# limacv/VideoLoop3D

Hardware: AMD Instinct MI355X
Metric: rendered Mpix/s (fwd+bwd) D=32 planes 720p (higher is better)
Workload: dtype f32; 1 GPU; cfg3 stage-2 MPV render fwd+bwd: D=32 planes, T=50 frames, 720x1280, mpv convention, plane stack (D,T,H,W,4) f32 resident in HBM; parallelism=single GPU, variant=0

## Files before the change

### profiles/ab_inproc.py

```python
#!/usr/bin/env python3
import argparse
import os
import statistics
import sys

sys.path.insert(0, os.path.dirname(os.path.dirname(os.path.abspath(__file__))))
import torch

ap = argparse.ArgumentParser()
ap.add_argument("--variants", default="0,3")
ap.add_argument("--rounds", type=int, default=6)
ap.add_argument("--reps", type=int, default=4)
ap.add_argument("--stack-scale", type=float, default=1.0)
ap.add_argument("--reg", action="store_true", help="smoothness regularisers on (the REG backward)")
ap.add_argument("--dtype", default="f32")
ap.add_argument("--D", type=int, default=32)
ap.add_argument("--T", type=int, default=50)
ap.add_argument("--H", type=int, default=720)
ap.add_argument("--W", type=int, default=1280)
a = ap.parse_args()

import __graft_entry__ as ge
ge.build()
from videoloop3d_amd import synth
from videoloop3d_amd.render import RenderSpec, render_planes, render_planes_with_smoothness
from videoloop3d_amd.utils_mpi import compute_homography, make_depths

dev = torch.device("cuda:0")
D, T, H, W = a.D, a.T, a.H, a.W
Hs, Ws = int(H * a.stack_scale), int(W * a.stack_scale)
ref_e, Kr, tar_e, Kt = synth.make_cameras(H, W)
homos = compute_homography(ref_e[None], Kr[None], tar_e[None], Kt[None], torch.tensor([0., 0., 1.]).expand(1, D, 3),
                           make_depths(D, 1.0, 100.0).flip(0)[None])[0]
shift = torch.tensor([[1.0, 0, (Ws - W) // 2], [0, 1.0, (Hs - H) // 2], [0, 0, 1.0]])
homos_d = (shift @ homos).to(dev)
stack = synth.make_plane_stack(D, T, Hs, Ws, seed=2, device=dev, dtype=torch.float16 if a.dtype == "f16" else torch.float32).requires_grad_(True)
g = synth.hash_uniform((T, H, W, 3), seed=5, device=dev) - 0.5
variants = [int(v, 0) for v in a.variants.split(",")]
ev = lambda: torch.cuda.Event(enable_timing=True)
res = [([], []) for _ in variants]


def once(v):
    spec = RenderSpec.mpv(variant=v)
    e0, e1, e2 = ev(), ev(), ev()
    e0.record()
    if a.reg:
        rgb, alpha, sums = render_planes_with_smoothness(stack, homos_d, H, W, spec)
        obj = (rgb * g).sum() + 1e-6 * sums.sum()
        e1.record()
        (gs,) = torch.autograd.grad(obj, stack)
    else:
        rgb, alpha = render_planes(stack, homos_d, H, W, spec)
        e1.record()
        (gs,) = torch.autograd.grad(rgb, stack, g)
    e2.record()
    torch.cuda.synchronize()
    once.last = gs
    return e0.elapsed_time(e1), e1.elapsed_time(e2)


g_first = None
for v in variants:
    once(v)
    if g_first is None:
        g_first = once.last.clone() if T <= 4 else None
    elif T <= 4:
        print(f"variant {v:#x}: gradient bits equal to variant {variants[0]:#x}: {torch.equal(g_first, once.last)}")
for r in range(a.rounds):
    for i, v in enumerate(variants):
        for _ in range(a.reps):
            f, b = once(v)
            res[i][0].append(f)
            res[i][1].append(b)
print(f"D={D} T={T} {H}x{W} stack {Hs}x{Ws} {a.dtype} reg={a.reg}: {a.rounds} rounds x {a.reps} reps, interleaved")
bmed = [statistics.median(b) for _, b in res]
for i, v in enumerate(variants):
    f, b = res[i]
    print(f"variant {v:#6x}  fwd median {statistics.median(f):7.3f} min {min(f):7.3f}   bwd median {bmed[i]:7.3f} min {min(b):7.3f} ms"
          + (f"   bwd vs leg 0: {100.0 * (bmed[i] / bmed[0] - 1.0):+6.2f} %" if i else ""))
spread = max([abs(bmed[i] - bmed[j]) for i in range(len(variants)) for j in range(i) if variants[i] == variants[j]], default=None)
if spread is not None:
    print(f"spread (backward medians of the legs that repeat a variant): {spread:.3f} ms = {100.0 * spread / bmed[0]:.2f} %; a gain counts from 3x that: {3 * spread:.3f} ms")
```

### videoloop3d_amd/csrc/vl3d_render_core.h

```cpp
#pragma once
#include <stddef.h>
#include "vl3d_common.h"
#include "vl3d_bake_rule.h"

#include "vl3d_adam.h"
#include "vl3d_render_bwd_choice.h"

#ifndef VL3D_HS
#define VL3D_HS 9
#define VL3D_HN 9
#endif

namespace vl3d_render_detail {

#ifndef VL3D_PAIR_MIN_WAVES
#define VL3D_PAIR_MIN_WAVES 4
#endif
#ifndef VL3D_FWD2X_MIN_WAVES
#define VL3D_FWD2X_MIN_WAVES 4
#endif

#ifdef VL3D_REG_ABLATE
#define VL3D_REGAB(bit) ((VL3D_REG_ABLATE & (bit)) != 0)
#else
// ... 565 lines not shown
    const float S = dot3p(Gr, a.rgb[pix * 3 + 0], Gg, a.rgb[pix * 3 + 1], Gb, a.rgb[pix * 3 + 2], gA * a.alpha[pix]);
    const float gN1 = a.g_asum ? a.g_asum[pix * 2 + 0] : 0.0f, gN2 = a.g_asum ? 2.0f * a.g_asum[pix * 2 + 1] : 0.0f;
    const unsigned fl = a.g_reg ? a.reg_flags[(size_t)y * a.W + x] : 0u;
    float Tr = 1.0f, P = 0.0f;
    const TapStep st = make_tap_step<F16>(a.Hs, a.Ws), gst = make_tap_step<false>(a.Hs, a.Ws);
    const float gL = MASK ? a.g_label[pix] : 0.0f;
    const size_t mframe = (size_t)a.Hs * a.Ws;
    for (int d = 0; d < a.D; ++d, plane += (size_t)a.T * a.Hs * a.Ws * TEXB, gplane += (size_t)a.T * a.Hs * a.Ws * TEXB) {
        const Taps2 tp = make_taps2<COORD, BORDER>(a.homos + VL3D_HS * d, px, py, a.Hs, a.Ws, a.sx, a.sy, a.ox, a.oy, plane_cull(a, d), UvNoise{a.uv_seed, d});
        if (tp.cov == 0.0f) continue;
        typename TapVal<F16, ORDER>::type tv[4];
        f4 pre;
        load_taps2<F16>(plane, tp, st, tv);
        const f4 o = shade2<ORDER, RACT, AACT>(tp, tv, &pre);
        const float q = dot3p(Gr, o.x, Gg, o.y, Gb, o.z, gA);
        const float w = o.w * Tr;
        if constexpr (MASK) {
            float mt[4];
            load_mask_taps(a.mask + ((size_t)d * a.T + t) * mframe, tp.off, gst, mt);
            const float sm = act_fwd<VL3D_ACT_SIGMOID>(mask_blend(mt, tp.w));
            const float gm = gL * w * (sm * (1.0f - sm));
            float *gmp = a.g_mask + ((size_t)d * a.T + t) * mframe + (tp.off >> 4);
#pragma unroll
            for (int i = 0; i < 4; ++i)
                if (tp.w[i] != 0.0f) atomicAdd(gmp + ((i & 1) ? (gst.dx >> 4) : 0u) + ((i & 2) ? (gst.dy >> 4) : 0u), gm * tp.w[i]);
        }
        P = fmaf(w, q, P);
        const float om = 1.0f - o.w;
        const float behind = (om > 1e-12f) ? (S - P) * fast_rcp(om) : 0.0f;
        f4 go = f4{w * Gr, w * Gg, w * Gb, fmaf(Tr, q, -behind) + fmaf(gN2, o.w, gN1)};
        Tr *= om;
        if (a.g_reg) {
            const f4 gx = f4{a.g_reg[0], a.g_reg[0], a.g_reg[0], a.g_reg[2]}, gy = f4{a.g_reg[1], a.g_reg[1], a.g_reg[1], a.g_reg[3]};
            const size_t idx = (((((size_t)(d >> 2) * a.T + t) * a.H + y) * a.W + x) << 2) + (d & 3);
            const unsigned w_left = x >= 1 ? a.reg_signs[idx - 4] : REG_ZERO, w_up = y >= 1 ? a.reg_signs[idx - 4 * (size_t)a.W] : REG_ZERO;
            go += reg_grad(a.reg_signs[idx], w_left, w_up, (fl & 12u) ? a.reg_patch[idx] : 0u, fl, gx, gy);
        }
        if constexpr (ORDER == VL3D_ACT_POST)
            go = f4{go.x * act_bwd<RACT>(pre.x, o.x), go.y * act_bwd<RACT>(pre.y, o.y), go.z * act_bwd<RACT>(pre.z, o.z),
                    go.w * act_bwd<AACT>(pre.w, o.w)};
#pragma unroll
        for (int i = 0; i < 4; ++i) {
            if (tp.w[i] != 0.0f) {
                f4 c = go * tp.w[i];
                if constexpr (ORDER == VL3D_ACT_PRE || ORDER == VL3D_ACT_BAKED) {
                    const f4 sv = tv[i];
                    c = f4{c.x * act_bwd<RACT>(sv.x, act_fwd<RACT>(sv.x)), c.y * act_bwd<RACT>(sv.y, act_fwd<RACT>(sv.y)),
                           c.z * act_bwd<RACT>(sv.z, act_fwd<RACT>(sv.z)), c.w * act_bwd<AACT>(sv.w, act_fwd<AACT>(sv.w))};
                }
                atomic_add_grad_texel<F16>(gplane, (size_t)tp.off + ((i & 1) ? gst.dx : 0u) + ((i & 2) ? gst.dy : 0u), c);
            }
        }
    }
}

__device__ __forceinline__ int xcd_remap(int b, int nb) {
    const int q = nb >> 3, r = nb & 7, xcd = b & 7, k = b >> 3;
    return (xcd < r ? xcd * (q + 1) : r * (q + 1) + (xcd - r) * q) + k;
}

template <int COORD, bool CAMS = false>
__global__ __launch_bounds__(256) void cull_fwd_plan_k(RenderArgs a, int TY, int tiles_x, int tiles_y, unsigned long long *masks) {
    const int i = blockIdx.x * 256 + threadIdx.x;
    if (i >= tiles_x * tiles_y * a.D) return;
    const int d = i % a.D, tile = i / a.D, tile_x = tile % tiles_x, tile_y = tile / tiles_x;
    const int x0 = tile_x * 64, x1 = min(x0 + 63, a.W - 1), y0 = tile_y * TY, y1 = min(y0 + TY - 1, a.H - 1);
    const float *h = a.homos + VL3D_HS * d;
    if constexpr (CAMS) {
        h += (size_t)blockIdx.y * a.D * VL3D_HS;
        masks += (size_t)blockIdx.y * tiles_x * tiles_y * 2;
    }
    float tnx = 1e30f, txx = -1e30f, tny = 1e30f, txy = -1e30f;
    for (int c = 0; c < 4; ++c) {
        const float cx = (float)a.col0 + a.pc + (float)((c & 1) ? x1 : x0), cy = (float)a.row0 + a.pc + (float)((c & 2) ? y1 : y0);
        const float X = h[0] * cx + h[1] * cy + h[2], Y = h[3] * cx + h[4] * cy + h[5], Z = h[6] * cx + h[7] * cy + h[8];
        const float ctx = texel_coord<COORD>(X / Z, (float)a.Ws / 2.0f, (float)(a.Ws - 1), a.sx, a.ox);
        const float cty = texel_coord<COORD>(Y / Z, (float)a.Hs / 2.0f, (float)(a.Hs - 1), a.sy, a.oy);
        tnx = fminf(tnx, ctx); txx = fmaxf(txx, ctx); tny = fminf(tny, cty); txy = fmaxf(txy, cty);
    }
    if (box_touches_kept_quad(a, d, tnx, txx, tny, txy)) atomicOr(masks + (size_t)tile * 2 + (d >> 6), 1ull << (d & 63));
}

template <int COORD>
void launch_cull_fwd_plan(const RenderArgs &a, int TY, int tiles_x, int tiles_y, hipStream_t s) {
    auto *masks = const_cast<unsigned long long *>(a.cull_masks);
    (void)hipMemsetAsync(masks, 0, (size_t)tiles_x * tiles_y * 16, s);
    const int n = tiles_x * tiles_y * a.D;
    hipLaunchKernelGGL((cull_fwd_plan_k<COORD>), dim3((n + 255) / 256), dim3(256), 0, s, a, TY, tiles_x, tiles_y, masks);
}
template <int COORD>
void launch_cull_fwd_plan_cams(const RenderArgs &a, int n_cams, int TY, int tiles_x, int tiles_y, hipStream_t s) {
    auto *masks = const_cast<unsigned long long *>(a.cull_masks);
    (void)hipMemsetAsync(masks, 0, (size_t)n_cams * tiles_x * tiles_y * 16, s);
    const int n = tiles_x * tiles_y * a.D;
    hipLaunchKernelGGL((cull_fwd_plan_k<COORD, true>), dim3((n + 255) / 256, n_cams), dim3(256), 0, s, a, TY, tiles_x, tiles_y, masks);
}

struct PlaneList {
    unsigned long long m0, m1;
    __device__ __forceinline__ PlaneList(const unsigned long long *cull_masks, int tile) {
        typedef const __attribute__((address_space(4))) unsigned long long *cu64_p;
        const cu64_p mk = (cu64_p)(cull_masks + (size_t)tile * 2);
        m0 = mk[0]; m1 = mk[1];
    }
    __device__ __forceinline__ int next() {
        int d = -1;
        if (m0) { d = __builtin_ctzll(m0); m0 &= m0 - 1; }
        else if (m1) { d = 64 + __builtin_ctzll(m1); m1 &= m1 - 1; }
        return d;
    }
};

template <int COORD, int BORDER, int ORDER, int RACT, int AACT, int TY, bool SWZ, bool F16, bool CULL = false, bool MASK = false>
__global__ __launch_bounds__(64 * TY) void render_fwd2_k(RenderArgs a, int tiles_x, int tiles_y) {
    static_assert(!(MASK && (CULL || F16)), "the loop-mask channel: dense fp32 stage-1 stacks");
    int b = blockIdx.x;
    if constexpr (SWZ) b = xcd_remap(b, gridDim.x);
    const int tile_x = b % tiles_x, rest = b / tiles_x;
    const int tile_y = rest % tiles_y, t = rest / tiles_y;
    const int x = tile_x * 64 + (threadIdx.x & 63);
    const int y = tile_y * TY + (threadIdx.x >> 6);
    if (x >= a.W || y >= a.H) return;
    const float px = (float)(a.col0 + x) + a.pc, py = (float)(a.row0 + y) + a.pc;
    const size_t frame_b = (size_t)a.Hs * a.Ws * (F16 ? 8 : 16);
    const size_t plane_stride_b = (size_t)a.Tstride * frame_b;
    const char *plane = reinterpret_cast<const char *>(a.stack) + (size_t)t * frame_b;
    float Tr = 1.0f, cr = 0.f, cg = 0.f, cb = 0.f, A = 0.f, n1 = 0.f, n2 = 0.f;
    const TapStep st = make_tap_step<F16>(a.Hs, a.Ws);
    typedef typename TapVal<F16, ORDER>::type tapv_t;
    tapv_t vA[4], vB[4];
    float mA[4] = {0.f, 0.f, 0.f, 0.f}, mB[4] = {0.f, 0.f, 0.f, 0.f}, lab = 0.f;
    const float *mplane = MASK ? a.mask + (size_t)t * a.Hs * a.Ws : nullptr;
    const size_t mplane_stride = (size_t)a.T * a.Hs * a.Ws;
#define VL3D_COMPOSITE(T_, V_, M_)                                    \
    {                                                                 \
        const f4 o = shade2<ORDER, RACT, AACT>(T_, V_);               \
        const float w = o.w * Tr;                                     \
        cr += w * o.x; cg += w * o.y; cb += w * o.z; A += w;          \
        n1 += o.w; n2 = fmaf(o.w, o.w, n2);                           \
        Tr *= (1.0f - o.w);                                           \
        if constexpr (MASK) lab = fmaf(w, act_fwd<VL3D_ACT_SIGMOID>(mask_blend(M_, T_.w)), lab);      \
    }
    if constexpr (CULL) {
        PlaneList list(a.cull_masks, tile_y * tiles_x + tile_x);
        auto fetch = [&](int d, Taps2 &t, tapv_t *v) {
            float h[VL3D_HN];
            load_uniform(a.homos + VL3D_HS * d, h);
            t = make_taps2<COORD, BORDER>(h, px, py, a.Hs, a.Ws, a.sx, a.sy, a.ox, a.oy, plane_cull(a, d), UvNoise{a.uv_seed, d});
            load_taps2<F16>(plane + (size_t)d * plane_stride_b, t, st, v);
            asm volatile("" ::: "memory");
        };
        int dA = list.next();
        if (dA >= 0) {
            Taps2 tA, tB;
            fetch(dA, tA, vA);
            for (;;) {
                const int dB = list.next();
                fetch(dB < 0 ? dA : dB, tB, vB);
                VL3D_COMPOSITE(tA, vA, mA)
                if (dB < 0) break;
                const int dC = list.next();
                fetch(dC < 0 ? dB : dC, tA, vA);
                VL3D_COMPOSITE(tB, vB, mB)
                if (dC < 0) break;
                dA = dC;
            }
        }
    } else {
    const QuadCull noq = QuadCull{nullptr, 0, 0, 0.f, 0.f, 0.f, 0.f, 0};
    Taps2 tA = make_taps2<COORD, BORDER>(a.homos, px, py, a.Hs, a.Ws, a.sx, a.sy, a.ox, a.oy, noq, UvNoise{a.uv_seed, 0}), tB = tA;
    load_taps2<F16>(plane, tA, st, vA);
    if constexpr (MASK) load_mask_taps(mplane, tA.off, st, mA);
    for (int d = 0;; d += 2) {
        {
            const int dn = min(d + 1, a.D - 1);
            float h[VL3D_HN];
            load_uniform(a.homos + VL3D_HS * dn, h);
            tB = make_taps2<COORD, BORDER>(h, px, py, a.Hs, a.Ws, a.sx, a.sy, a.ox, a.oy, noq, UvNoise{a.uv_seed, dn});
            load_taps2<F16>(plane + (size_t)dn * plane_stride_b, tB, st, vB);
            if constexpr (MASK) load_mask_taps(mplane + (size_t)dn * mplane_stride, tB.off, st, mB);
            asm volatile("" ::: "memory");
        }
        VL3D_COMPOSITE(tA, vA, mA)
        if (d + 1 >= a.D) break;
        {
            const int dn = min(d + 2, a.D - 1);
            float h[VL3D_HN];
            load_uniform(a.homos + VL3D_HS * dn, h);
            tA = make_taps2<COORD, BORDER>(h, px, py, a.Hs, a.Ws, a.sx, a.sy, a.ox, a.oy, noq, UvNoise{a.uv_seed, dn});
            load_taps2<F16>(plane + (size_t)dn * plane_stride_b, tA, st, vA);
            if constexpr (MASK) load_mask_taps(mplane + (size_t)dn * mplane_stride, tA.off, st, mA);
            asm volatile("" ::: "memory");
        }
        VL3D_COMPOSITE(tB, vB, mB)
        if (d + 2 >= a.D) break;
    }
    }
#undef VL3D_COMPOSITE
    const size_t pix = ((size_t)t * a.H + y) * a.W + x;
    a.rgb[pix * 3 + 0] = cr; a.rgb[pix * 3 + 1] = cg; a.rgb[pix * 3 + 2] = cb;
    a.alpha[pix] = A;
    if (a.asum) { a.asum[pix * 2 + 0] = n1; a.asum[pix * 2 + 1] = n2; }
    if constexpr (MASK) a.label[pix] = lab;
}

template <int COORD, int BORDER, int ORDER, int RACT, int AACT, int TY, bool F16, bool CULL = false>
__global__ __launch_bounds__(64 * TY, VL3D_FWD2X_MIN_WAVES) void render_fwd2x_k(RenderArgs a, int tiles_x, int tiles_y) {
    const int b = xcd_remap(blockIdx.x, gridDim.x);
    const int tile_x = b % tiles_x, rest = b / tiles_x;
    const int tile_y = rest % tiles_y, t0 = (rest / tiles_y) * 2;
    const bool has1 = t0 + 1 < a.T;
    const int x = tile_x * 64 + (threadIdx.x & 63);
    const int y = tile_y * TY + (threadIdx.x >> 6);
    if (x >= a.W || y >= a.H) return;
    const float px = (float)(a.col0 + x) + a.pc, py = (float)(a.row0 + y) + a.pc;
    const size_t frame_b = (size_t)a.Hs * a.Ws * (F16 ? 8 : 16);
    const size_t plane_stride_b = (size_t)a.Tstride * frame_b;
    const char *plane0 = reinterpret_cast<const char *>(a.stack) + (size_t)t0 * frame_b;
    const char *plane1 = plane0 + (has1 ? frame_b : 0);
    float Tr0 = 1.0f, cr0 = 0.f, cg0 = 0.f, cb0 = 0.f, A0 = 0.f, n10 = 0.f, n20 = 0.f;
    float Tr1 = 1.0f, cr1 = 0.f, cg1 = 0.f, cb1 = 0.f, A1 = 0.f, n11 = 0.f, n21 = 0.f;
    const TapStep st = make_tap_step<F16>(a.Hs, a.Ws);
    typedef typename TapVal<F16, ORDER>::type tapv_t;
    tapv_t vA0[4], vA1[4], vB0[4], vB1[4];
#define VL3D_COMPOSITE2(T_, V0_, V1_)                                        \
    {                                                                        \
        const f4 o0 = shade2<ORDER, RACT, AACT>(T_, V0_);                    \
        const f4 o1 = shade2<ORDER, RACT, AACT>(T_, V1_);                    \
        const float w0 = o0.w * Tr0, w1 = o1.w * Tr1;                        \
        cr0 += w0 * o0.x; cg0 += w0 * o0.y; cb0 += w0 * o0.z; A0 += w0;      \
        cr1 += w1 * o1.x; cg1 += w1 * o1.y; cb1 += w1 * o1.z; A1 += w1;      \
        n10 += o0.w; n20 = fmaf(o0.w, o0.w, n20);                            \
        n11 += o1.w; n21 = fmaf(o1.w, o1.w, n21);                            \
        Tr0 *= (1.0f - o0.w); Tr1 *= (1.0f - o1.w);                          \
    }
    if constexpr (CULL) {
        PlaneList list(a.cull_masks, tile_y * tiles_x + tile_x);
        auto fetch = [&](int d, Taps2 &t, tapv_t *v0, tapv_t *v1) {
            float h[VL3D_HN];
            load_uniform(a.homos + VL3D_HS * d, h);
            t = make_taps2<COORD, BORDER>(h, px, py, a.Hs, a.Ws, a.sx, a.sy, a.ox, a.oy, plane_cull(a, d));
            load_taps2<F16>(plane0 + (size_t)d * plane_stride_b, t, st, v0);
            load_taps2<F16>(plane1 + (size_t)d * plane_stride_b, t, st, v1);
            asm volatile("" ::: "memory");
        };
        int dA = list.next();
        if (dA >= 0) {
            Taps2 tA, tB;
            fetch(dA, tA, vA0, vA1);
            for (;;) {
                const int dB = list.next();
                fetch(dB < 0 ? dA : dB, tB, vB0, vB1);
                VL3D_COMPOSITE2(tA, vA0, vA1)
                if (dB < 0) break;
                const int dC = list.next();
                fetch(dC < 0 ? dB : dC, tA, vA0, vA1);
                VL3D_COMPOSITE2(tB, vB0, vB1)
                if (dC < 0) break;
                dA = dC;
            }
        }
    } else {
    Taps2 tA = make_taps2<COORD, BORDER>(a.homos, px, py, a.Hs, a.Ws, a.sx, a.sy, a.ox, a.oy), tB = tA;
    load_taps2<F16>(plane0, tA, st, vA0);
    load_taps2<F16>(plane1, tA, st, vA1);
    for (int d = 0;; d += 2) {
        {
            const int dn = min(d + 1, a.D - 1);
            float h[VL3D_HN];
            load_uniform(a.homos + VL3D_HS * dn, h);
            tB = make_taps2<COORD, BORDER>(h, px, py, a.Hs, a.Ws, a.sx, a.sy, a.ox, a.oy);
            load_taps2<F16>(plane0 + (size_t)dn * plane_stride_b, tB, st, vB0);
            load_taps2<F16>(plane1 + (size_t)dn * plane_stride_b, tB, st, vB1);
            asm volatile("" ::: "memory");
        }
        VL3D_COMPOSITE2(tA, vA0, vA1)
        if (d + 1 >= a.D) break;
        {
            const int dn = min(d + 2, a.D - 1);
            float h[VL3D_HN];
            load_uniform(a.homos + VL3D_HS * dn, h);
            tA = make_taps2<COORD, BORDER>(h, px, py, a.Hs, a.Ws, a.sx, a.sy, a.ox, a.oy);
            load_taps2<F16>(plane0 + (size_t)dn * plane_stride_b, tA, st, vA0);
            load_taps2<F16>(plane1 + (size_t)dn * plane_stride_b, tA, st, vA1);
            asm volatile("" ::: "memory");
        }
        VL3D_COMPOSITE2(tB, vB0, vB1)
        if (d + 2 >= a.D) break;
    }
    }
#undef VL3D_COMPOSITE2
    size_t pix = ((size_t)t0 * a.H + y) * a.W + x;
    a.rgb[pix * 3 + 0] = cr0; a.rgb[pix * 3 + 1] = cg0; a.rgb[pix * 3 + 2] = cb0;
    a.alpha[pix] = A0;
    if (a.asum) { a.asum[pix * 2 + 0] = n10; a.asum[pix * 2 + 1] = n20; }
    if (has1) {
        pix += (size_t)a.H * a.W;
        a.rgb[pix * 3 + 0] = cr1; a.rgb[pix * 3 + 1] = cg1; a.rgb[pix * 3 + 2] = cb1;
        a.alpha[pix] = A1;
        if (a.asum) { a.asum[pix * 2 + 0] = n11; a.asum[pix * 2 + 1] = n21; }
    }
}

template <int COORD, int BORDER, int ORDER, int RACT, int AACT, bool F16>
void launch_fwd2x(const RenderArgs &a, hipStream_t s) {
    constexpr int TY = 8;
    const int tiles_x = (a.W + 63) / 64, tiles_y = (a.H + TY - 1) / TY;
    const dim3 grid((unsigned)(tiles_x * tiles_y * ((a.T + 1) / 2))), block(64 * TY);
    if (a.quad_keep && a.cull_masks) {
        launch_cull_fwd_plan<COORD>(a, TY, tiles_x, tiles_y, s);
        hipLaunchKernelGGL((render_fwd2x_k<COORD, BORDER, ORDER, RACT, AACT, TY, F16, true>), grid, block, 0, s, a, tiles_x, tiles_y);
        return;
    }
    hipLaunchKernelGGL((render_fwd2x_k<COORD, BORDER, ORDER, RACT, AACT, TY, F16>), grid, block, 0, s, a, tiles_x, tiles_y);
}

template <int COORD, int BORDER, int ORDER, int RACT, int AACT, int TY, bool SWZ, bool F16 = false>
void launch_fwd2(const RenderArgs &a, hipStream_t s) {
    const int tiles_x = (a.W + 63) / 64, tiles_y = (a.H + TY - 1) / TY;
    if (a.quad_keep && a.cull_masks) {
        launch_cull_fwd_plan<COORD>(a, TY, tiles_x, tiles_y, s);
        hipLaunchKernelGGL((render_fwd2_k<COORD, BORDER, ORDER, RACT, AACT, TY, SWZ, F16, true>), dim3((unsigned)(tiles_x * tiles_y * a.T)),
                           dim3(64 * TY), 0, s, a, tiles_x, tiles_y);
        return;
    }
    hipLaunchKernelGGL((render_fwd2_k<COORD, BORDER, ORDER, RACT, AACT, TY, SWZ, F16>), dim3((unsigned)(tiles_x * tiles_y * a.T)),
                       dim3(64 * TY), 0, s, a, tiles_x, tiles_y);
}

constexpr int RW = 64;
constexpr int PLAN_HDR = 16;
constexpr int PLAN_REC = 12;
__host__ __device__ inline int plan_win_off(int D) { return (PLAN_HDR + PLAN_REC * D + 3) & ~3; }

template <int COORD>
__device__ void texel_homography(const float *h, int Hs, int Ws, float sx, float sy, float ox, float oy, double M[9]) {
    double ax, ay, bx, by;
    if constexpr (COORD == VL3D_COORD_UTILS_MPI) { ax = (double)(Ws - 1) / Ws; ay = (double)(Hs - 1) / Hs; bx = by = 0.0; }
    else { ax = sx; ay = sy; bx = ox; by = oy; }
    for (int j = 0; j < 3; ++j) {
        M[0 + j] = ax * h[0 + j] + bx * h[6 + j];
        M[3 + j] = ay * h[3 + j] + by * h[6 + j];
        M[6 + j] = h[6 + j];
    }
}

template <int COORD>
__global__ void bwd_plan_k(RenderArgs a, int rows, float *plan) {
    __shared__ int ok_all;
    if (threadIdx.x == 0) ok_all = 1;
    __syncthreads();
    for (int d = threadIdx.x; d < a.D; d += blockDim.x) {
        double M[9];
        texel_homography<COORD>(a.homos + VL3D_HS * d, a.Hs, a.Ws, a.sx, a.sy, a.ox, a.oy, M);
        const double det = M[0] * (M[4] * M[8] - M[5] * M[7]) - M[1] * (M[3] * M[8] - M[5] * M[6]) +
                           M[2] * (M[3] * M[7] - M[4] * M[6]);
        bool ok = (det == det) && fabs(det) > 1e-30;
        double I[9];
        I[0] = (M[4] * M[8] - M[5] * M[7]) / det; I[1] = (M[2] * M[7] - M[1] * M[8]) / det; I[2] = (M[1] * M[5] - M[2] * M[4]) / det;
        I[3] = (M[5] * M[6] - M[3] * M[8]) / det; I[4] = (M[0] * M[8] - M[2] * M[6]) / det; I[5] = (M[2] * M[3] - M[0] * M[5]) / det;
        I[6] = (M[3] * M[7] - M[4] * M[6]) / det; I[7] = (M[1] * M[6] - M[0] * M[7]) / det; I[8] = (M[0] * M[4] - M[1] * M[3]) / det;
        for (int i = 0; i < 9; ++i) plan[PLAN_HDR + PLAN_REC * d + i] = (float)I[i];
        double rxm = 0.0, rym = 0.0;
        for (int gy = 0; gy < 3 && ok; ++gy)
            for (int gx = 0; gx < 3 && ok; ++gx) {
                const double x = a.col0 + a.pc + (gx == 0 ? -2.0 : (gx == 1 ? 0.5 * a.W : a.W + 1.0));
                const double y = a.row0 + a.pc + (gy == 0 ? -2.0 : (gy == 1 ? 0.5 * a.H : a.H + 1.0));
                const double X = M[0] * x + M[1] * y + M[2], Y = M[3] * x + M[4] * y + M[5], Z = M[6] * x + M[7] * y + M[8];
                if (!(Z > 1e-20)) { ok = false; break; }
                const double j00 = (M[0] * Z - X * M[6]) / (Z * Z), j01 = (M[1] * Z - X * M[7]) / (Z * Z);
                const double j10 = (M[3] * Z - Y * M[6]) / (Z * Z), j11 = (M[4] * Z - Y * M[7]) / (Z * Z);
                const double dj = j00 * j11 - j01 * j10;
                if (!(fabs(dj) > 1e-12)) { ok = false; break; }
                const double i_r0 = (fabs(j11) + fabs(j01)) / fabs(dj), i_r1 = (fabs(j10) + fabs(j00)) / fabs(dj);
                if (!(i_r0 < 1.4 && i_r1 < 1.4)) ok = false;
                rxm = fmax(rxm, i_r0); rym = fmax(rym, i_r1);
                if (!(fabs(j00) + fabs(j01) < 4.0 && fabs(j10) + fabs(j11) < 4.0)) ok = false;
            }
        plan[PLAN_HDR + PLAN_REC * d + 9] = (float)fmin(1.02 * rxm + 1e-3, 1.45);
        plan[PLAN_HDR + PLAN_REC * d + 10] = (float)fmin(1.02 * rym + 1e-3, 1.45);
        if (!ok) atomicAnd(&ok_all, 0);
    }
    __syncthreads();
    if (threadIdx.x == 0) { reinterpret_cast<int *>(plan)[0] = ok_all; reinterpret_cast<int *>(plan)[1] = 0; }
    if (threadIdx.x < 4) plan[4 + threadIdx.x] = 0.0f;
    if (threadIdx.x >= 8 && threadIdx.x < 16) plan[threadIdx.x] = 0.0f;
    if (threadIdx.x == 2 || threadIdx.x == 3) plan[threadIdx.x] = 0.0f;
}

template <int COORD>
__global__ __launch_bounds__(256) void bwd_windows_k(RenderArgs a, int iw, int ih, int rh, int tiles_x, int tiles_y, int *win) {
    const int i = blockIdx.x * 256 + threadIdx.x;
    if (i >= tiles_x * tiles_y * a.D) return;
    const int d = i % a.D, tile = i / a.D, tile_x = tile % tiles_x, tile_y = tile / tiles_x;
    const int ix0 = tile_x * iw, ix1 = min(ix0 + iw - 1, a.W - 1), iy0 = tile_y * ih, iy1 = min(iy0 + ih - 1, a.H - 1);
    const float el = (ix0 == 0) ? 1.6f : 0.55f, er = (ix1 == a.W - 1) ? 1.6f : 0.55f;
    const float et = (iy0 == 0) ? 1.6f : 0.55f, eb = (iy1 == a.H - 1) ? 1.6f : 0.55f;
    const float *h = a.homos + VL3D_HS * d;
    float mnx = 1e30f, mxx = -1e30f, mny = 1e30f, mxy = -1e30f;
    for (int c = 0; c < 4; ++c) {
        const float cx = (float)a.col0 + a.pc + ((c & 1) ? (float)ix1 + er : (float)ix0 - el);
        const float cy = (float)a.row0 + a.pc + ((c & 2) ? (float)iy1 + eb : (float)iy0 - et);
        const float X = h[0] * cx + h[1] * cy + h[2], Y = h[3] * cx + h[4] * cy + h[5], Z = h[6] * cx + h[7] * cy + h[8];
        const float ctx = texel_coord<COORD>(X / Z, (float)a.Ws / 2.0f, (float)(a.Ws - 1), a.sx, a.ox);
        const float cty = texel_coord<COORD>(Y / Z, (float)a.Hs / 2.0f, (float)(a.Hs - 1), a.sy, a.oy);
        mnx = fminf(mnx, ctx); mxx = fmaxf(mxx, ctx); mny = fminf(mny, cty); mxy = fmaxf(mxy, cty);
    }
    if (a.q_th) {
        const float qlo_x = fminf(fmaxf(ceilf((mnx - 0.01f + a.q_x0) * a.q_inv_cw - 1e-3f) - 1.0f, 0.0f), (float)(a.QW - 1));
        const float qhi_x = fminf(fmaxf(floorf((mxx + 0.01f + a.q_x0) * a.q_inv_cw + 1e-3f), 0.0f), (float)(a.QW - 1));
        const float qlo_y = fminf(fmaxf(ceilf((mny - 0.01f + a.q_y0) * a.q_inv_ch - 1e-3f) - 1.0f, 0.0f), (float)(a.QH - 1));
        const float qhi_y = fminf(fmaxf(floorf((mxy + 0.01f + a.q_y0) * a.q_inv_ch + 1e-3f), 0.0f), (float)(a.QH - 1));
        mnx += qlo_x; mxx += qhi_x; mny += qlo_y; mxy += qhi_y;
    }
    const int wX0 = max(0, (int)ceilf(fmaxf(mnx - 0.01f, -2.0f))), wY0 = max(0, (int)ceilf(fmaxf(mny - 0.01f, -2.0f)));
    const int wX1 = min(a.Ws - 1, (int)floorf(fminf(mxx + 0.01f, (float)a.Ws)));
    const int wY1 = min(a.Hs - 1, (int)floorf(fminf(mxy + 0.01f, (float)a.Hs)));
    const int ww = min(max(0, wX1 - wX0 + 1), 0xffff), wh = min(max(0, wY1 - wY0 + 1), 0x3fff);
    int4 rec;
    const bool empty = ww == 0 || wh == 0;
    rec.x = empty ? 0 : wX0; rec.y = empty ? 0 : wY0; rec.z = empty ? 0 : (ww | (wh << 16)); rec.w = __float_as_int(1.0f / (float)max(ww, 1));
    {
        float ax, ay;
        if constexpr (COORD == VL3D_COORD_UTILS_MPI) { ax = (float)(a.Ws - 1) / (float)a.Ws; ay = (float)(a.Hs - 1) / (float)a.Hs; }
        else { ax = a.sx; ay = a.sy; }
        bool apart = !a.gather9;
        for (int c = 0; c < 4; ++c) {
            const float cx = (float)a.col0 + a.pc + (float)((c & 1) ? tile_x * iw + iw - 1 + rh + 1 : ix0 - rh - 1);
            const float cy = (float)a.row0 + a.pc + (float)((c & 2) ? tile_y * ih + ih - 1 + rh + 1 : iy0 - rh - 1);
            const float X = h[0] * cx + h[1] * cy + h[2], Y = h[3] * cx + h[4] * cy + h[5], Z = h[6] * cx + h[7] * cy + h[8];
            const float iz2 = 1.0f / (Z * Z);
            const float j00 = ax * (h[0] * Z - X * h[6]) * iz2, j01 = ax * (h[1] * Z - X * h[7]) * iz2;
            const float j10 = ay * (h[3] * Z - Y * h[6]) * iz2, j11 = ay * (h[4] * Z - Y * h[7]) * iz2;
            apart = apart && (Z > 0.0f) && (j00 - fabsf(j01) >= 1.001f) && (j11 - fabsf(j10) >= 1.001f);
        }
        if (apart && !empty) rec.z |= 0x40000000;
    }
    if (a.quad_keep) {
        const int qx0 = max(ix0 - rh, 0), qx1 = min(tile_x * iw + iw - 1 + rh, a.W - 1);
        const int qy0 = max(iy0 - rh, 0), qy1 = min(tile_y * ih + ih - 1 + rh, a.H - 1);
        float tnx = 1e30f, txx = -1e30f, tny = 1e30f, txy = -1e30f;
        for (int c = 0; c < 4; ++c) {
            const float cx = (float)a.col0 + a.pc + (float)((c & 1) ? qx1 : qx0), cy = (float)a.row0 + a.pc + (float)((c & 2) ? qy1 : qy0);
            const float X = h[0] * cx + h[1] * cy + h[2], Y = h[3] * cx + h[4] * cy + h[5], Z = h[6] * cx + h[7] * cy + h[8];
            const float ctx = texel_coord<COORD>(X / Z, (float)a.Ws / 2.0f, (float)(a.Ws - 1), a.sx, a.ox);
            const float cty = texel_coord<COORD>(Y / Z, (float)a.Hs / 2.0f, (float)(a.Hs - 1), a.sy, a.oy);
            tnx = fminf(tnx, ctx); txx = fmaxf(txx, ctx); tny = fminf(tny, cty); txy = fmaxf(txy, cty);
        }
        if (!box_touches_kept_quad(a, d, tnx, txx, tny, txy)) rec.z |= (int)0x80000000;
    }
    reinterpret_cast<int4 *>(win)[i] = rec;
}

__device__ __forceinline__ void lattice_texel(const RenderArgs &a, int x, int y, float &lx, float &ly) {
    lx = (float)x; ly = (float)y;
    if (a.q_th) {
        lx -= fminf(floorf(((float)x + a.q_x0 + 0.5f) * (1.0f / (float)a.q_tw)), (float)(a.QW - 1));
        ly -= fminf(floorf(((float)y + a.q_y0 + 0.5f) * (1.0f / (float)a.q_th)), (float)(a.QH - 1));
    }
}

__device__ __forceinline__ void owner_pixel(const float *__restrict__ hi, float tx, float ty, float pc, int col0, int row0,
                                            float &px, float &py) {
    const float X = hi[0] * tx + hi[1] * ty + hi[2];
    const float Y = hi[3] * tx + hi[4] * ty + hi[5];
    const float Z = hi[6] * tx + hi[7] * ty + hi[8];
    const float rz = fast_rcp(Z);
    px = X * rz - pc - (float)col0;
    py = Y * rz - pc - (float)row0;
}

__device__ __forceinline__ bool adam_texel(const RenderArgs &a, int d, int cx, int cy, int &from, unsigned &off) {
    const int X = a.ad.x0 + cx, Y = a.ad.y0 + cy;
    if (a.ad.boxes) {
        const cint_p b = (cint_p)a.ad.boxes + 4 * d;
        if (Y < b[0] || Y >= b[1] || X < b[2] || X >= b[3]) return false;
    }
    static_assert(vl3d_adam::TS == 8, "bookkeeping tiles of 8 x 8 texels");
    from = a.ad.last_step[((size_t)d * a.ad.tiles_y + (Y >> 3)) * a.ad.tiles_x + (X >> 3)];
    off = (unsigned)(Y * a.ad.Ws + X) << 4;
    return true;
}
__device__ __forceinline__ void adam_texel_inbox(const RenderArgs &a, int d, int cx, int cy, int &from, size_t &off) {
    const int X = a.ad.x0 + cx, Y = a.ad.y0 + cy;
    const size_t tile = ((size_t)d * a.ad.tiles_y + (Y >> 3)) * a.ad.tiles_x + (X >> 3);
    from = a.ad.last_step[tile];
    if (a.ad.blocks) off = ((size_t)(a.ad.blocks[tile] >> 1) * 64 + (size_t)((Y & 7) * 8 + (X & 7))) << 4;
    else off = (size_t)((unsigned)(Y * a.ad.Ws + X) << 4);
}
__device__ __forceinline__ size_t adam_frame_base(const RenderArgs &a, int d, int t) {
    return a.ad.blocks ? (size_t)t * 1024 : ((size_t)d * a.T + t) * ((size_t)a.ad.Hs * a.ad.Ws * 16);
}
template <typename OFF>
__device__ __forceinline__ void adam_texel_step_mv(const RenderArgs &a, size_t fb, OFF off, int from, f4 pcur, f4 g, f4 m0, f4 v0) {
    char *pb = reinterpret_cast<char *>(a.ad.p) + fb, *mb = reinterpret_cast<char *>(a.ad.m) + fb, *vb = reinterpret_cast<char *>(a.ad.v) + fb;
    float4 mm = make_float4(m0.x, m0.y, m0.z, m0.w), vv = make_float4(v0.x, v0.y, v0.z, v0.w);
    vl3d_adam::replay_moments(mm, vv, from, a.ad.step - 1, a.ad.beta1, a.ad.beta2);
    float4 pp = make_float4(pcur.x, pcur.y, pcur.z, pcur.w);
    vl3d_adam::adam_upd4(pp, make_float4(g.x, g.y, g.z, g.w), mm, vv, a.ad.lr_bc1, a.ad.beta1, a.ad.beta2, a.ad.eps, a.ad.bc2s);
    __builtin_nontemporal_store(f4{pp.x, pp.y, pp.z, pp.w}, reinterpret_cast<f4 *>(pb + (size_t)off));
    __builtin_nontemporal_store(f4{mm.x, mm.y, mm.z, mm.w}, reinterpret_cast<f4 *>(mb + (size_t)off));
    __builtin_nontemporal_store(f4{vv.x, vv.y, vv.z, vv.w}, reinterpret_cast<f4 *>(vb + (size_t)off));
}
template <typename OFF>
__device__ __forceinline__ void adam_texel_step(const RenderArgs &a, size_t fb, OFF off, int from, f4 pcur, f4 g) {
    const char *mb = reinterpret_cast<const char *>(a.ad.m) + fb, *vb = reinterpret_cast<const char *>(a.ad.v) + fb;
    adam_texel_step_mv(a, fb, off, from, pcur, g, *reinterpret_cast<const f4 *>(mb + (size_t)off), *reinterpret_cast<const f4 *>(vb + (size_t)off));
}

__global__ __launch_bounds__(256) void bwd_owner_table_k(RenderArgs a, int iw, int ih, int rh, int tiles_x, unsigned short *owner, int rw = 64,
                                                         int slot_bits = 10) {
    if (!reinterpret_cast<const int *>(a.plan)[0]) return;
    const int x = blockIdx.x * 64 + (threadIdx.x & 63);
    const int y = blockIdx.y * 4 + (threadIdx.x >> 6);
    const int d = blockIdx.z;
    if (x >= a.Ws || y >= a.Hs) return;
    float qx, qy, lx, ly;
    lattice_texel(a, x, y, lx, ly);
    owner_pixel(a.plan + PLAN_HDR + PLAN_REC * d, lx, ly, a.pc, a.col0, a.row0, qx, qy);
    const float rxf = fminf(fmaxf(rintf(qx), 0.0f), (float)(a.W - 1)), ryf = fminf(fmaxf(rintf(qy), 0.0f), (float)(a.H - 1));
    const int rx = (int)rxf, ry = (int)ryf;
    const int tx = (int)((rxf + 0.5f) * (1.0f / (float)iw)), ty = (int)((ryf + 0.5f) * (1.0f / (float)ih));
    const unsigned lc = (unsigned)((ry - ty * ih + rh) * rw + (rx - tx * iw + rh));
    const unsigned ymask = slot_bits == 9 ? 15u : 7u;
    const unsigned ent = ((((unsigned)ty & ymask) << 3 | (unsigned)(tx & 7)) << slot_bits) | lc;
    const unsigned e1 = __shfl_down(ent, 1, 64), e2 = __shfl_down(ent, 2, 64), e3 = __shfl_down(ent, 3, 64);
    unsigned short *dst = owner + ((size_t)d * a.Hs + y) * a.Ws + x;
    if ((a.Ws & 3) == 0 && x + 3 < a.Ws) {
        if ((threadIdx.x & 3) == 0) *reinterpret_cast<uint2 *>(dst) = make_uint2(ent | e1 << 16, e2 | e3 << 16);
    } else {
        *dst = (unsigned short)ent;
    }
    int cls = 1;
    if (a.ad.p && a.ad.cls) {
        const int X = a.ad.x0 + x, Y = a.ad.y0 + y;
        bool inbox = true;
        if (a.ad.boxes) {
            const cint_p b = (cint_p)a.ad.boxes + 4 * d;
            inbox = !(Y < b[0] || Y >= b[1] || X < b[2] || X >= b[3]);
        }
        cls = inbox ? vl3d_adam::texel_class(vl3d_adam::Quads{a.quad_keep, a.ad.quad_dyn, a.QH, a.QW, a.q_th, a.q_tw}, d, X, Y, a.ad.Hs, a.ad.Ws) : 3;
        int rfrom = 0;
        size_t roff = 0;
        if (cls == 1) adam_texel_inbox(a, d, x, y, rfrom, roff);
        a.ad.cls[((size_t)d * a.Hs + y) * a.Ws + x] = make_uint2((unsigned)cls | ((unsigned)rfrom << 2), (unsigned)(roff >> 4));
    }
    const bool safe = (qx > 0.5f) && (qx < (float)a.W - 1.5f) && (qy > 0.5f) && (qy < (float)a.H - 1.5f);
    if (safe) return;
    const size_t frame = (size_t)a.Hs * a.Ws;
    if (a.ad.p) {
        const int4 rec = reinterpret_cast<const int4 *>(reinterpret_cast<const int *>(a.plan) + plan_win_off(a.D))[(size_t)(ty * tiles_x + tx) * a.D + d];
        const int ww = rec.z & 0xffff, wh = (rec.z >> 16) & 0x3fff;
        if (rec.z >= 0 && x >= rec.x && x < rec.x + ww && y >= rec.y && y < rec.y + wh) return;
        int from;
        unsigned off;
        if (cls == 2) {
            float4 *g = reinterpret_cast<float4 *>(a.g_stack) + (size_t)d * a.T * frame + (size_t)y * a.Ws + x;
            for (int t = 0; t < a.T; ++t, g += frame) *g = make_float4(0.f, 0.f, 0.f, 0.f);
            return;
        }
        if (cls != 1) return;
        const f4 *pc = reinterpret_cast<const f4 *>(a.stack) + (size_t)d * a.T * frame + (size_t)y * a.Ws + x;
        if (a.ad.cls) {
            size_t offp;
            adam_texel_inbox(a, d, x, y, from, offp);
            for (int t = 0; t < a.T; ++t, pc += frame) adam_texel_step(a, adam_frame_base(a, d, t), offp, from, *pc, f4{0.f, 0.f, 0.f, 0.f});
            return;
        }
        if (!adam_texel(a, d, x, y, from, off)) return;
        for (int t = 0; t < a.T; ++t, pc += frame) adam_texel_step(a, adam_frame_base(a, d, t), off, from, *pc, f4{0.f, 0.f, 0.f, 0.f});
        return;
    }
    if (a.g_f16) {
        float2 *g = reinterpret_cast<float2 *>(a.g_stack) + (size_t)d * a.T * frame + (size_t)y * a.Ws + x;
        for (int t = 0; t < a.T; ++t, g += frame) *g = make_float2(0.f, 0.f);
    } else {
        float4 *g = reinterpret_cast<float4 *>(a.g_stack) + (size_t)d * a.T * frame + (size_t)y * a.Ws + x;
        for (int t = 0; t < a.T; ++t, g += frame) *g = make_float4(0.f, 0.f, 0.f, 0.f);
    }
    if (a.g_mask) {
        float *g = a.g_mask + (size_t)d * a.T * frame + (size_t)y * a.Ws + x;
        for (int t = 0; t < a.T; ++t, g += frame) *g = 0.f;
    }
}

__global__ __launch_bounds__(256) void bwd_owner_table4_k(RenderArgs a, int iw, int ih, int rh, unsigned short *owner, int rw, int slot_bits) {
    if (!reinterpret_cast<const int *>(a.plan)[0]) return;
    const int x0 = (blockIdx.x * 64 + (threadIdx.x & 63)) * 4;
    const int y = blockIdx.y * 4 + (threadIdx.x >> 6);
    const int d = blockIdx.z;
    if (x0 >= a.Ws || y >= a.Hs) return;
    const float *hi = a.plan + PLAN_HDR + PLAN_REC * d;
    const unsigned ymask = slot_bits == 9 ? 15u : 7u;
    const float inv_iw = 1.0f / (float)iw, inv_ih = 1.0f / (float)ih;
    unsigned ent[4];
    bool unsafe[4];
#pragma unroll
    for (int k = 0; k < 4; ++k) {
        float qx, qy, lx, ly;
        lattice_texel(a, x0 + k, y, lx, ly);
        owner_pixel(hi, lx, ly, a.pc, a.col0, a.row0, qx, qy);
        const float rxf = fminf(fmaxf(rintf(qx), 0.0f), (float)(a.W - 1)), ryf = fminf(fmaxf(rintf(qy), 0.0f), (float)(a.H - 1));
        const int rx = (int)rxf, ry = (int)ryf;
        const int tx = (int)((rxf + 0.5f) * inv_iw), ty = (int)((ryf + 0.5f) * inv_ih);
        const unsigned lc = (unsigned)((ry - ty * ih + rh) * rw + (rx - tx * iw + rh));
        ent[k] = ((((unsigned)ty & ymask) << 3 | (unsigned)(tx & 7)) << slot_bits) | lc;
        unsafe[k] = !((qx > 0.5f) && (qx < (float)a.W - 1.5f) && (qy > 0.5f) && (qy < (float)a.H - 1.5f));
    }
    const size_t row = ((size_t)d * a.Hs + y) * a.Ws;
    unsigned short *dst = owner + row + x0;
    if ((a.Ws & 3) == 0) {
        *reinterpret_cast<uint2 *>(dst) = make_uint2(ent[0] | ent[1] << 16, ent[2] | ent[3] << 16);
    } else {
#pragma unroll
        for (int k = 0; k < 4; ++k)
// ... 851 lines not shown
```

Before: 2753 Mpix/s.

## Add row-pair forward kernel sharing bilinear taps between vertically adjacent pixels

Adds a forward render kernel where each thread composites two vertically adjacent pixels of one frame. The lower pixel reuses the upper pixel's bottom texel row when its tap offset is exactly one row below, and only loads its own top row when that fails. This replaces the two-frames-per-thread fwd2x path for f32 in most configurations, aiming to cut texel fetches. It costs extra registers, a wave-wide ballot branch per plane, and the reuse only pays off when the homographies keep adjacent rows one texel row apart.

```diff
diff --git a/profiles/ab_inproc.py b/profiles/ab_inproc.py
--- a/profiles/ab_inproc.py
+++ b/profiles/ab_inproc.py
@@ -82,3 +82,7 @@
 spread = max([abs(bmed[i] - bmed[j]) for i in range(len(variants)) for j in range(i) if variants[i] == variants[j]], default=None)
 if spread is not None:
     print(f"spread (backward medians of the legs that repeat a variant): {spread:.3f} ms = {100.0 * spread / bmed[0]:.2f} %; a gain counts from 3x that: {3 * spread:.3f} ms")
+    fmed = [statistics.median(f) for f, _ in res]
+    fspread = max(abs(fmed[i] - fmed[j]) for i in range(len(variants)) for j in range(i) if variants[i] == variants[j])
+    print("forward medians against leg 0: " + "  ".join(f"{v:#x} {fmed[i] - fmed[0]:+.3f} ms" for i, v in enumerate(variants) if i)
+          + f"; spread of the repeated legs {fspread:.3f} ms = {100.0 * fspread / fmed[0]:.2f} %")
diff --git a/videoloop3d_amd/csrc/vl3d_render_core.h b/videoloop3d_amd/csrc/vl3d_render_core.h
--- a/videoloop3d_amd/csrc/vl3d_render_core.h
+++ b/videoloop3d_amd/csrc/vl3d_render_core.h
@@ -891,6 +891,94 @@
     }
 }
 
+struct Taps2R {
+    Taps2 u, l;
+    unsigned off2;
+    bool own;
+};
+template <int COORD, int BORDER, int ORDER, int RACT, int AACT>
+__global__ __launch_bounds__(512, 4) void render_fwd2r_k(RenderArgs a, int tiles_x, int tiles_y) {
+    const int b = xcd_remap(blockIdx.x, gridDim.x);
+    const int tile_x = b % tiles_x, rest = b / tiles_x;
+    const int tile_y = rest % tiles_y, t = rest / tiles_y;
+    const int x = tile_x * 64 + (threadIdx.x & 63);
+    const int y = tile_y * 16 + (int)(threadIdx.x >> 6) * 2;
+    if (x >= a.W || y >= a.H) return;
+    const bool hasL = y + 1 < a.H;
+    const float px = (float)(a.col0 + x) + a.pc, pyU = (float)(a.row0 + y) + a.pc, pyL = (float)(a.row0 + y + 1) + a.pc;
+    const size_t frame_b = (size_t)a.Hs * a.Ws * 16;
+    const size_t plane_stride_b = (size_t)a.Tstride * frame_b;
+    const char *plane = reinterpret_cast<const char *>(a.stack) + (size_t)t * frame_b;
+    float TrU = 1.0f, crU = 0.f, cgU = 0.f, cbU = 0.f, AU = 0.f, n1U = 0.f, n2U = 0.f;
+    float TrL = 1.0f, crL = 0.f, cgL = 0.f, cbL = 0.f, AL = 0.f, n1L = 0.f, n2L = 0.f;
+    const TapStep st = make_tap_step<false>(a.Hs, a.Ws);
+    Taps2R tA, tB;
+    f4 vA[6], vB[6];
+    auto fetch = [&](int d, Taps2R &tp, f4 *v) {
+        float h[VL3D_HN];
+        load_uniform(a.homos + VL3D_HS * d, h);
+        tp.u = make_taps2<COORD, BORDER>(h, px, pyU, a.Hs, a.Ws, a.sx, a.sy, a.ox, a.oy);
+        tp.l = make_taps2<COORD, BORDER>(h, px, pyL, a.Hs, a.Ws, a.sx, a.sy, a.ox, a.oy);
+        tp.own = hasL && tp.l.off != tp.u.off + st.dy;
+        tp.off2 = hasL ? tp.l.off : tp.u.off;
+        const char *__restrict__ p = plane + (size_t)d * plane_stride_b;
+        v[0] = load_texel<false>(p, tp.u.off);
+        v[1] = load_texel<false>(p + st.dx, tp.u.off);
+        v[2] = load_texel<false>(p + st.dy, tp.u.off);
+        v[3] = load_texel<false>(p + st.dy + st.dx, tp.u.off);
+        v[4] = load_texel<false>(p + st.dy, tp.off2);
+        v[5] = load_texel<false>(p + st.dy + st.dx, tp.off2);
+        asm volatile("" ::: "memory");
+    };
+#define VL3D_COMPOSITE1(O_, S_)                                                                     \
+    {                                                                                               \
+        const float w = O_.w * Tr##S_;                                                              \
+        cr##S_ += w * O_.x; cg##S_ += w * O_.y; cb##S_ += w * O_.z; A##S_ += w;                     \
+        n1##S_ += O_.w; n2##S_ = fmaf(O_.w, O_.w, n2##S_);                                          \
+        Tr##S_ *= (1.0f - O_.w);                                                                    \
+    }
+#define VL3D_COMPOSITE2R(T_, V_, D_)                                                                \
+    {                                                                                               \
+        const f4 oU = shade2<ORDER, RACT, AACT>(T_.u, V_);                                          \
+        VL3D_COMPOSITE1(oU, U)                                                                      \
+        f4 oL;                                                                                      \
+        if (__builtin_amdgcn_ballot_w64(T_.own) != 0ull) {                                          \
+            f4 vl[4] = {V_[2], V_[3], V_[4], V_[5]};                                                \
+            if (T_.own) {                                                                           \
+                const char *__restrict__ p = plane + (size_t)(D_) * plane_stride_b;                 \
+                vl[0] = load_texel<false>(p, T_.l.off);                                             \
+                vl[1] = load_texel<false>(p + st.dx, T_.l.off);                                     \
+            }                                                                                       \
+            oL = shade2<ORDER, RACT, AACT>(T_.l, vl);                                               \
+            asm volatile("; render_fwd2r_k own taps" ::: "memory");                                 \
+        } else {                                                                                    \
+            oL = shade2<ORDER, RACT, AACT>(T_.l, V_ + 2);                                           \
+        }                                                                                           \
+        VL3D_COMPOSITE1(oL, L)                                                                      \
+    }
+    fetch(0, tA, vA);
+    for (int d = 0;; d += 2) {
+        fetch(min(d + 1, a.D - 1), tB, vB);
+        VL3D_COMPOSITE2R(tA, vA, d)
+        if (d + 1 >= a.D) break;
+        fetch(min(d + 2, a.D - 1), tA, vA);
+        VL3D_COMPOSITE2R(tB, vB, d + 1)
+        if (d + 2 >= a.D) break;
+    }
+#undef VL3D_COMPOSITE2R
+#undef VL3D_COMPOSITE1
+    const size_t pix = ((size_t)t * a.H + y) * a.W + x;
+    a.rgb[pix * 3 + 0] = crU; a.rgb[pix * 3 + 1] = cgU; a.rgb[pix * 3 + 2] = cbU;
+    a.alpha[pix] = AU;
+    if (a.asum) { a.asum[pix * 2 + 0] = n1U; a.asum[pix * 2 + 1] = n2U; }
+    if (hasL) {
+        const size_t pl = pix + a.W;
+        a.rgb[pl * 3 + 0] = crL; a.rgb[pl * 3 + 1] = cgL; a.rgb[pl * 3 + 2] = cbL;
+        a.alpha[pl] = AL;
+        if (a.asum) { a.asum[pl * 2 + 0] = n1L; a.asum[pl * 2 + 1] = n2L; }
+    }
+}
+
 template <int COORD, int BORDER, int ORDER, int RACT, int AACT, bool F16>
 void launch_fwd2x(const RenderArgs &a, hipStream_t s) {
     constexpr int TY = 8;
@@ -900,6 +988,13 @@
         launch_cull_fwd_plan<COORD>(a, TY, tiles_x, tiles_y, s);
         hipLaunchKernelGGL((render_fwd2x_k<COORD, BORDER, ORDER, RACT, AACT, TY, F16, true>), grid, block, 0, s, a, tiles_x, tiles_y);
         return;
+    }
+    if constexpr (!F16 && !(ORDER == VL3D_ACT_PRE && BORDER == VL3D_BORDER_HARDCUT)) {
+        if (a.fwd_variant != 7) {
+            const int tiles_y2 = (a.H + 15) / 16;
+            hipLaunchKernelGGL((render_fwd2r_k<COORD, BORDER, ORDER, RACT, AACT>), dim3((unsigned)(tiles_x * tiles_y2 * a.T)), dim3(512), 0, s, a, tiles_x, tiles_y2);
+            return;
+        }
     }
     hipLaunchKernelGGL((render_fwd2x_k<COORD, BORDER, ORDER, RACT, AACT, TY, F16>), grid, block, 0, s, a, tiles_x, tiles_y);
 }
```

Result: faster. 2867 Mpix/s, median of 6 (+4.1%).
